# KyleVanMeter/MVOLPS

Measured on AMD Instinct MI355X. Metric: simplex_pivots_per_s, higher is better.
Workload: dtype f64

## Files before the change

mvolps_amd/csrc/engine.cpp:

```cpp
#include <hip/hip_runtime.h>

#include <cmath>
#include <cstdio>
#include <cstdlib>
#include <cstring>
#include <atomic>
#include <limits>
#include <map>
#include <mutex>
#include <tuple>
#include <unordered_map>
#include <unordered_set>
#include <vector>

#include "engine.hpp"

struct DevMatrix {
  int m0 = 0, n = 0, lda = 0;
  double *plain = nullptr, *packed = nullptr;
  int *len = nullptr;
  std::vector<const void *> rows;
  ~DevMatrix() {
    if (packed && packed != plain) (void)hipFree(packed);
    if (plain) (void)hipFree(plain);
    if (len) (void)hipFree(len);
  }
};

struct RoundModel {
  int m0 = 0, n = 0, ldm = 0, dir = 0;
  void *dev = nullptr;
  void *dev_rows = nullptr;
  int ldn = 0;
  size_t o_rlo = 0, o_rhi = 0, o_clo = 0, o_chi = 0, o_c = 0, o_flags = 0;
  std::vector<mvx::RowPtr> rows;
  std::vector<double> c, clb, cub, rlb, rub;
  std::vector<int> kind;
  ~RoundModel() {
    if (dev) (void)hipFree(dev);
    if (dev_rows) (void)hipFree(dev_rows);
  }
};

namespace mvx {

#define HIPCHECK(expr)                                                                         \
  do {                                                                                         \
    hipError_t e_ = (expr);                                                                    \
    if (e_ != hipSuccess) {                                                                    \
      std::fprintf(stderr, "mvx: HIP error %s at %s:%d (%s)\n", hipGetErrorString(e_), __FILE__, __LINE__, #expr); \
      std::abort();                                                                            \
    }                                                                                          \
  } while (0)

void set_tuning(int tr, int hot, int nt);
int fused_npb(int n);
int fused_nrb_max(int m);
int chain_ncb(int n);
int chain_nrb(int m);
void launch_pboot(const ChainArgs &, hipStream_t);
void launch_pstep(const ChainArgs &, int g, hipStream_t);
void launch_pc(const ChainArgs &, int g, hipStream_t);
void launch_fbc3(const ChainArgs &, int steps, hipStream_t);
void launch_fpatch(const ChainArgs &, int steps, hipStream_t);
int launch_chain(const ChainArgs &, hipStream_t);
int chain_cluster_nw(int m, int n);
int chain_cluster_kmax(int m, int n);
void launch_dboot(Ctl *, int n, hipStream_t);
void launch_da(Ctl *, int n, hipStream_t);
void launch_db(Ctl *, int m, int n, hipStream_t);
void launch_select(Ctl *, hipStream_t, int slots = 1);
int launch_dsel(Ctl *, int m, int n, hipStream_t, int slots = 1);
void launch_select_queue(Ctl *, const BatchQueue &q, hipStream_t, int slots);
void launch_update(Ctl *, int m, int n, hipStream_t, int slots = 1, int chained = 0, int busy_slots = 0);
void launch_p1_head(Ctl *, hipStream_t);
void launch_p1_select(Ctl *, hipStream_t);
void launch_p1_fix(Ctl *, int n, hipStream_t);
void launch_scatter_ctl(Ctl *dst, const Ctl *src, const int *idx, int count, hipStream_t);
void launch_copy_many(const CopyBatch &b, hipStream_t);
void launch_gmi(const GmiArgs &a, hipStream_t);
void launch_classify(const ClsArgs &a, hipStream_t);
void launch_penalty(const PenArgs &a, hipStream_t);
void launch_round(const RndArgs &a, hipStream_t);
void launch_rcfix(const RcArgs &a, hipStream_t);
void launch_tighten(const TightHandle *hs, const TightEntry *es, int count, hipStream_t);
void launch_prop(const PropArgs &a, hipStream_t);
void launch_setbnds(const SetbHandle *hs, const SetbEntry *es, const SetbShift *ss, int handles, hipStream_t);
void launch_refresh_select(Ctl *, const int *tflag, int var, hipStream_t);
size_t persist_lds_bytes(int m, int cpw);
int persist_max_cpw();
int persist_slot_words(int m_cap);
int launch_persist(Ctl *, unsigned long long *head, unsigned long long *slot, int *abort_flag, unsigned long long *dbg, int m, int cpw, int nw,
                   int slot_stride, int max_steps, int head_stride, hipStream_t);
void launch_rowcomb(Ctl *, int m, int n, int respect_done, hipStream_t);
void launch_shift_nonbasic(double *T, int ld, int m, int jj, double delta, hipStream_t);
void launch_set_basic_bounds(double *blb, double *bub, int i, double lb, double ub, hipStream_t);
void launch_set_nonbasic(double *nlb, double *nub, int *nflag, int j, double lb, double ub, int flag, hipStream_t);
void launch_add_rows(double *T, int ld, int n, int *bvar, double *blb, double *bub, int *nvar, int first, int nrs, int m_new,
                     hipStream_t);
void launch_export(Ctl *, unsigned char *stage, int m, int n, int force, hipStream_t, int slots = 1, size_t slot_stride = 0);

static inline size_t align_up(size_t x, size_t a) { return (x + a - 1) / a * a; }

struct Carver {
  size_t off = 0;
  size_t operator()(size_t bytes) {
    size_t o = off;
    off = align_up(off + bytes, 256);
    return o;
  }
};

constexpr size_t XG_BYTES = 4 * 8 * 64 * 16;
struct SolveCtx {
  hipStream_t stream = nullptr;
  Ctl *d_ctl = nullptr;
  Ctl *h_ctl = nullptr;
  int sc_m_cap = 0, sc_ld = 0;
  void *scratch = nullptr;
  double *d_colq = nullptr, *d_srow = nullptr, *d_cost1 = nullptr, *d_wts = nullptr, *d_part = nullptr, *d_rcbase = nullptr;
  int *d_gflag = nullptr;
  double *d_colqx[2] = {nullptr, nullptr}, *d_betac[2] = {nullptr, nullptr};
  double *d_dw = nullptr, *d_dw2 = nullptr;
  int *d_p1list = nullptr;
  int *d_tflag = nullptr;
  double *d_pw[2] = {nullptr, nullptr};
  double *d_srowk[KCH] = {}, *d_colqk[KCH] = {};
  double *d_drowk[2] = {}, *d_pwk[2] = {}, *d_nlbk[2] = {}, *d_nubk[2] = {}, *d_betak[2] = {}, *d_blbk[2] = {}, *d_bubk[2] = {};
  int *d_nflagk[2] = {};
  double *d_betab = nullptr, *d_ppart = nullptr, *d_rpart = nullptr;
  double *d_zeros = nullptr;
  unsigned char *rc_ring = nullptr;
  size_t rc_slot_bytes = 0;
  int rc_next = 0, rc_m_cap = 0, rc_ld = 0;
  unsigned *d_xg = nullptr;
  int *d_xabort = nullptr;
  unsigned xtag = 0;
  size_t pp_stride = 0, rp_stride = 0;
  size_t sk_stride = 0, ck_stride = 0;
  Cand *d_rpc = nullptr;
  double *d_olb = nullptr, *d_oub = nullptr;
  Cand *d_pp[2] = {nullptr, nullptr}, *d_rp = nullptr;
  unsigned char *d_stage = nullptr, *h_stage = nullptr;
  bool stage_zc = false;
  size_t stage_bytes = 0;
  hipEvent_t ev_a = nullptr, ev_b = nullptr;
  unsigned long long *d_pcand = nullptr, *d_pmsg = nullptr;
// ... 892 lines not shown
  if (J.parm.it_lim > 8 && J.try_fused) J.batch = std::min(J.parm.it_lim, 256);
}

static void job_enqueue(Context &c, SolveJob &J) {
  mvx_prob *P = J.P;
  SolveCtx &sc = *J.sc;
  const int m = P->m, n = P->n;
  J.ev_used = 0;
  if (J.mode == SolveJob::FINAL) {
    launch_export(sc.d_ctl, sc.d_stage, m, n, 1, sc.stream);
    stage_copy_async(sc, P);
    return;
  }
  if (J.mode == SolveJob::PHASE1) {
    for (int k = 0; k < J.pb; k++) {
      launch_p1_head(sc.d_ctl, sc.stream);
      launch_p1_fix(sc.d_ctl, n, sc.stream);
      launch_p1_select(sc.d_ctl, sc.stream);
      launch_update(sc.d_ctl, m + 1, n, sc.stream);
    }
    launch_export(sc.d_ctl, sc.d_stage, m, n, 0, sc.stream);
    stage_copy_async(sc, P);
    return;
  }
  const int batch = J.batch;
  if (J.profiled && c.ev_pool.size() < (size_t)2 * batch + 4) {
    size_t old = c.ev_pool.size();
    c.ev_pool.resize((size_t)2 * batch + 4);
    for (size_t k = old; k < c.ev_pool.size(); k++) HIPCHECK(hipEventCreate(&c.ev_pool[k]));
  }
  const int remaining = (J.parm.it_lim >= 0) ? std::max(0, J.parm.it_lim - J.seen_pivots) : (1 << 30);
  auto ev = [&]() {
    if (J.profiled) HIPCHECK(hipEventRecord(c.ev_pool[J.ev_used++], sc.stream));
  };
  int depth;
  if (J.try_fused) depth = std::max(0, std::min(batch, remaining));
  else depth = std::max(1, std::min(batch, remaining));
  auto body = [&](int m_grid) {
    if (J.try_fused) {
      PersistPlan pl;
      if (depth > 0 && !J.profiled && J.resident && !(J.cluster && !g_cluster_broken.load()) && persist_plan(c, P, &pl) && ensure_persist(c, sc, P, pl)) {
        launch_select(sc.d_ctl, sc.stream);
        launch_update(sc.d_ctl, m_grid, n, sc.stream, 1, 1);
        HIPCHECK(hipMemcpyAsync(sc.p_backup, P->slab, P->slab_bytes, hipMemcpyDeviceToDevice, sc.stream));
        HIPCHECK(hipMemcpyAsync(sc.d_pctl, sc.d_ctl, sizeof(Ctl), hipMemcpyDeviceToDevice, sc.stream));
        HIPCHECK(hipMemcpyAsync(sc.d_ppw, sc.d_pw[0], (size_t)P->ld * 8, hipMemcpyDeviceToDevice, sc.stream));
        HIPCHECK(hipMemcpyAsync(sc.d_ppw + P->ld, sc.d_pw[1], (size_t)P->ld * 8, hipMemcpyDeviceToDevice, sc.stream));
        const int head_stride = 4;
        HIPCHECK(hipMemsetAsync(sc.d_pcand, 0, (size_t)2 * pl.nw * head_stride * 8, sc.stream));
        const int steps = 1 << 24;
        if (launch_persist(sc.d_ctl, sc.d_pcand, sc.d_pmsg, sc.d_pabort, (unsigned long long *)(sc.d_pabort + 16), P->m, pl.cpw, pl.nw, sc.p_msg_words, steps, head_stride, sc.stream) == 0) {
          J.persist_queued = true;
          g_persist_launches++;
          launch_select(sc.d_ctl, sc.stream);
          launch_update(sc.d_ctl, m_grid, n, sc.stream, 1, 1);
        } else {
          g_persist_broken = true;
        }
      } else {
        const size_t e_generic = J.ev_used;
        if (J.profiled) J.ev_used += 2;
        if (depth > 0) {
          const bool cl = J.cluster && !g_cluster_broken.load();
          if (!cl) launch_pboot(J.cargs, sc.stream);
          bool first = true;
          const int kc = cl ? std::max(1, std::min(J.chain0, chain_cluster_kmax(m, n))) : std::max(1, J.chain);
          auto chain_launch = [&](int steps) {
            J.cargs.kmax = steps;
            J.cargs.boot = first ? 1 : 0;
            first = false;
            J.cargs.tagbase = sc.xtag;
            sc.xtag += 128;
            if (launch_chain(J.cargs, sc.stream) != 0) g_cluster_broken.store(true);
            g_cluster_launches++;
          };
          for (int left = depth; left > 0;) {
            const int steps = std::min(kc, left);
            if (cl) chain_launch(steps);
            else
              for (int t = 0; t < steps; t++) launch_pstep(J.cargs, t, sc.stream);
            ev();
            launch_fbc3(J.cargs, steps, sc.stream);
            ev();
            launch_fpatch(J.cargs, steps, sc.stream);
            left -= steps;
          }
          if (J.parm.it_lim >= 0 && depth >= remaining && !cl) launch_pc(J.cargs, 0, sc.stream);
        }
        launch_select(sc.d_ctl, sc.stream);
        if (J.profiled) HIPCHECK(hipEventRecord(c.ev_pool[e_generic], sc.stream));
        launch_update(sc.d_ctl, m_grid, n, sc.stream, 1, 1);
        if (J.profiled) HIPCHECK(hipEventRecord(c.ev_pool[e_generic + 1], sc.stream));
      }
    } else if (J.try_dfused) {
      launch_select(sc.d_ctl, sc.stream);
      launch_update(sc.d_ctl, m_grid, n, sc.stream, 1, 1);
      if (depth > 1) {
        launch_dboot(sc.d_ctl, n, sc.stream);
        launch_db(sc.d_ctl, m_grid, n, sc.stream);
        for (int k = 0; k < depth - 1; k++) {
          launch_da(sc.d_ctl, n, sc.stream);
          launch_db(sc.d_ctl, m_grid, n, sc.stream);
        }
      }
    } else {
      for (int k = 0; k < depth; k++) {
        launch_dsel(sc.d_ctl, m, n, sc.stream);
        launch_select(sc.d_ctl, sc.stream);
        ev();
        launch_update(sc.d_ctl, m_grid, n, sc.stream, 1, 1);
        ev();
      }
    }
    launch_export(sc.d_ctl, sc.d_stage, m_grid, n, 0, sc.stream);
    stage_copy_async(sc, P);
  };
  body(m);
}

static bool job_finalize(SolveJob &J) {
  mvx_prob *P = J.P;
  SolveCtx &sc = *J.sc;
  const Ctl &snap = J.snap;
  const unsigned char *s = sc.h_stage;
  const double *beta = (const double *)(s + sizeof(Ctl));
  const double *dj = beta + (P->m_cap + 1);
  const int *bv = (const int *)(dj + P->ld);
  const int *nv = bv + (P->m_cap + 1);
  const int *nf = nv + P->ld;
  P->beta.assign(beta, beta + P->m + 1);
  P->dj.assign(dj, dj + P->n + 1);
  P->bvar.assign(bv, bv + P->m + 1);
  P->nvar.assign(nv, nv + P->n + 1);
  P->nflag.assign(nf, nf + P->n + 1);
  rebuild_pos(P);
  P->sol_fresh = true;
  P->fresh_rows = -1;
  float ms = 0.f;
  HIPCHECK(hipEventElapsedTime(&ms, sc.ev_a, sc.ev_b));
  P->last_ms = ms;
  P->it_cnt += snap.it_cnt;
  P->bland_cnt += snap.n_bland;
  P->pert_cnt += snap.n_pert;
  P->hint_dual = false;
  switch (J.done) {
    case D_OPT: P->status = MVX_OPT; J.rc = 0; break;
    case D_UNBND: P->status = MVX_UNBND; J.rc = 0; break;
    case D_NOFEAS: P->status = MVX_NOFEAS; J.rc = 0; break;
    case D_ITLIM:
      P->status = (snap.phase == PH_PRIMAL2) ? MVX_FEAS : MVX_INFEAS;
      J.rc = MVX_EITLIM;
      break;
    default: P->status = MVX_UNDEF; J.rc = MVX_EFAIL; break;
  }
  return true;
}

static bool job_collect(Context &c, SolveJob &J) {
  SolveCtx &sc = *J.sc;
  Ctl &snap = J.snap;
  if (J.persist_queued) {
    J.persist_queued = false;
    if (sc.h_pabort[0]) {
      mvx_prob *P = J.P;
      g_persist_broken = true;
      g_persist_aborts++;
      std::fprintf(stderr, "mvx: resident-tableau launch aborted (workgroups not co-resident in time); using the two-kernel path from now on\n");
// ... 1662 lines not shown
```

mvolps_amd/csrc/kernels.hip:

```cpp
#include <hip/hip_runtime.h>

#include <cmath>
#include <cstdlib>

#include "mvx_internal.hpp"

namespace mvx {

#define TIDX ((int)threadIdx.x)

__device__ __forceinline__ double xdiv(double a, double b) {
  const double q = a / b;
  const double aq = fabs(q);
  if (!(aq > 1e-290 && aq < 1e290)) return q;
  const double r = fma(-q, b, a);
  if (r == 0.0) return q;
  const bool up = (r > 0.0) == (b > 0.0);
  long long bits = __double_as_longlong(q);
  bits += ((q > 0.0) == up) ? 1 : -1;
  const double q1 = __longlong_as_double(bits);
  const double r1 = fma(-q1, b, a);
  return (fabs(r1) < fabs(r)) ? q1 : q;
}

// ... 2628 lines not shown
      A.drowk[xf][0] = z;
      A.pwk[xf][0] = 1.0;
    }
  }
  if (lead) {
    c->pc_n = g;
    if (g > 0) {
      c->phase = PH_PRIMAL2;
      c->pc_itlim = end_itlim ? 1 : 0;
    }
  }
}

__device__ void chain_commit(const ChainArgs &A, Ctl *c, int nch) {
  __shared__ int s_cp[KCH], s_cq[KCH], s_ck[KCH], s_rf[KCH], s_cf[KCH], s_R[KCH], s_C[KCH];
  const int t = TIDX;
  const bool on = (t < nch);
  int kind = 0, p = 0, q = 0;
  if (on) {
    kind = c->ch_kind[t];
    p = c->ch_p[t];
    q = c->ch_q[t];
    s_ck[t] = kind;
    s_cp[t] = p;
    s_cq[t] = q;
    s_R[t] = (kind == ST_PIVOT) ? c->bvar[p] : 0;
    s_C[t] = (kind == ST_PIVOT) ? c->nvar[q] : 0;
  }
  __syncthreads();
  bool lastrow = true, lastcol = true, lastflag = true;
  if (on) {
    int rf = t, cf = t;
    for (int u = t - 1; u >= 0; u--) {
      if (s_ck[u] != ST_PIVOT) continue;
      if (s_cp[u] == p) rf = u;
      if (s_cq[u] == q) cf = u;
    }
    s_rf[t] = rf;
    s_cf[t] = cf;
    for (int u = t + 1; u < nch; u++) {
      if (s_cq[u] == q) lastflag = false;
      if (s_ck[u] != ST_PIVOT) continue;
      if (s_cp[u] == p) lastrow = false;
      if (s_cq[u] == q) lastcol = false;
    }
  }
  __syncthreads();
  if (t == 0) {
    for (int u = 0; u < nch; u++) {
      if (s_ck[u] != ST_PIVOT) continue;
      const int a = s_rf[u], b = s_cf[u];
      const int kv = s_R[a];
      s_R[a] = s_C[b];
      s_C[b] = kv;
    }
  }
  __syncthreads();
  if (on) {
    if (kind == ST_PIVOT) {
      if (lastrow) {
        c->bvar[p] = s_R[s_rf[t]];
        A.blb[p] = c->ch_elb[t];
        A.bub[p] = c->ch_eub[t];
      }
      if (lastcol) {
        c->nvar[q] = s_C[s_cf[t]];
        A.nlb[q] = c->ch_llb[t];
        A.nub[q] = c->ch_lub[t];
      }
    }
    if (lastflag) A.nflag[q] = c->ch_lf[t];
  }
  if (t == 0) {
    const int piv_n = c->ch_cnt[nch - 1];
    c->it_cnt += piv_n;
    c->n_flips += nch - piv_n;
    c->n_bulk++;
    if (c->budget > 0) c->budget -= piv_n;
    c->stall = c->ch_stall[nch - 1];
    c->pc_epoch++;
  }
}

typedef const double __attribute__((address_space(4))) *kconst_f64;
template <int TR, int NT>
__global__ __launch_bounds__(256) void k_fbc3(const ChainArgs A) {
  __shared__ double s_cq[KCH][TR];
  Ctl *const c = A.c;
  if (c->done != D_RUN || c->fstate != F_RUN) return;
  const int nch = c->pc_n;
  if (nch == 0) return;
  const int n = A.n;
  const size_t ld = (size_t)A.ld;
  const int j0 = 2 * ((int)blockIdx.x * 256 + TIDX);
  const int i0 = 1 + (int)blockIdx.y * TR;
  const int xf = nch & 1;
  const bool act = (j0 <= n);
  const int jc = act ? j0 : 0;
  double *base = A.T + (size_t)i0 * ld + jc;
  double2 v[TR];
#pragma unroll
  for (int r = 0; r < TR; r++) v[r] = ld2<NT>(reinterpret_cast<const double2 *>(base + (size_t)r * ld));
  unsigned flips = 0;
  for (int l = 0; l < nch; l++) flips |= (c->ch_kind[l] == ST_FLIP) ? (1u << l) : 0u;
  for (int e = TIDX; e < nch * TR; e += 256) {
    const int l = e / TR, r = e % TR;
    s_cq[l][r] = ((flips >> l) & 1u) ? 0.0 : A.colq0[(size_t)l * A.cstride + i0 + r];
  }
  __syncthreads();
  const double *sp = A.srow0 + jc;
  const double *zp = A.zeros + jc;
  for (int l0 = 0; l0 < nch; l0 += 4) {
    double2 s4[4];
#pragma unroll
    for (int k = 0; k < 4; k++) {
      const int lk = (l0 + k < nch) ? l0 + k : nch - 1;
      s4[k] = *reinterpret_cast<const double2 *>(((flips >> lk) & 1u) ? zp : sp + (size_t)lk * A.sstride);
    }
#pragma unroll
    for (int k = 0; k < 4; k++) {
      if (l0 + k < nch) {
#pragma unroll
        for (int r = 0; r < TR; r++) {
          const double ci = s_cq[l0 + k][r];
          asm("v_fma_f64 %0, -%1, %2, %0" : "+v"(v[r].x) : "v"(ci), "v"(s4[k].x));
          asm("v_fma_f64 %0, -%1, %2, %0" : "+v"(v[r].y) : "v"(ci), "v"(s4[k].y));
        }
      }
    }
  }
  if (act) {
    if (j0 == 0) {
#pragma unroll
      for (int r = 0; r < TR; r++) base[(size_t)r * ld + 1] = v[r].y;
    } else {
#pragma unroll
      for (int r = 0; r < TR; r++) st2<NT>(reinterpret_cast<double2 *>(base + (size_t)r * ld), v[r]);
    }
    if (blockIdx.y == 0) {
      *reinterpret_cast<double2 *>(A.T + j0) = *reinterpret_cast<const double2 *>(A.drowk[xf] + j0);
      const double2 w = *reinterpret_cast<const double2 *>(A.pwk[xf] + j0);
      *reinterpret_cast<double2 *>(A.pw[0] + j0) = w;
      *reinterpret_cast<double2 *>(A.pw[1] + j0) = w;
    }
  }
  if (blockIdx.x == 0 && blockIdx.y == 0) chain_commit(A, c, nch);
}

__global__ __launch_bounds__(256) void k_fpatch(const ChainArgs A, int kmax) {
  __shared__ int s_kind[KCH], s_p[KCH], s_q[KCH];
  __shared__ double s_piv[KCH], s_ip[KCH], s_xq[KCH], s_delta[KCH], s_u[KCH];
  Ctl *const c = A.c;
  if (c->done != D_RUN || c->fstate != F_RUN) return;
  const int nch = c->pc_n;
  if (nch == 0) return;
  const int m = A.m, n = A.n;
  const size_t ld = (size_t)A.ld;
  const int job = (int)blockIdx.y, x = (int)blockIdx.x * 256 + TIDX;
  const int jk = (job < kmax) ? 0 : (job < 2 * kmax) ? 1 : 2;
  const int l = (jk == 0) ? job : (jk == 1) ? job - kmax : -1;
  bool live = (jk == 2) || (l < nch && c->ch_kind[l < nch ? l : 0] == ST_PIVOT);
  const int span = (jk == 0) ? n : (jk == 1) ? m : A.mcap1 - 1;
  if ((int)blockIdx.x * 256 > span) live = false;
  if (live) {
    const int lp = (l >= 0) ? c->ch_p[l] : 0, lq = (l >= 0) ? c->ch_q[l] : 0;
    if (TIDX < KCH) {
      const int t = (TIDX < nch) ? TIDX : nch - 1;
      const int kind = c->ch_kind[t];
      const double piv = c->ch_piv[t];
      s_kind[TIDX] = kind;
      s_p[TIDX] = c->ch_p[t];
      s_q[TIDX] = c->ch_q[t];
      s_piv[TIDX] = piv;
      s_ip[TIDX] = (kind == ST_PIVOT) ? xdiv(1.0, piv) : 0.0;
      s_xq[TIDX] = c->ch_xq[t];
      s_delta[TIDX] = c->ch_delta[t];
      s_u[TIDX] = (jk == 0) ? A.colq0[(size_t)t * A.cstride + lp] : A.srow0[(size_t)t * A.sstride + (jk == 1 ? lq : 0)];
    }
    const int xc = (x >= 1 && x <= span) ? x : 1;
    double op[KCH];
#pragma unroll
    for (int t = 0; t < KCH; t++) {
      const int tc = (t < nch) ? t : nch - 1;
      op[t] = (jk == 0) ? A.srow0[(size_t)tc * A.sstride + xc] : A.colq0[(size_t)tc * A.cstride + xc];
    }
    double *dst = (jk == 0) ? A.T + (size_t)lp * ld + xc : A.T + (size_t)xc * ld + (jk == 1 ? lq : 0);
    double val = (jk == 2) ? *dst : 0.0;
    __syncthreads();
    const int i = (jk == 0) ? lp : xc, j = (jk == 0) ? xc : (jk == 1) ? lq : 0;
    const int l0 = (jk == 2) ? 0 : l;
#pragma unroll
    for (int t = 0; t < KCH; t++) {
      if (t >= l0 && t < nch) {
        const double ci = (jk == 0) ? s_u[t] : op[t], sj = (jk == 0) ? op[t] : s_u[t];
        if (s_kind[t] == ST_FLIP) {
          if (j == 0) val = fma(ci, s_delta[t], val);
        } else if (i == s_p[t]) {
          val = (j == s_q[t]) ? s_ip[t] : (j == 0) ? s_xq[t] - sj : -sj;
        } else if (j == s_q[t]) {
          val = xdiv(ci, s_piv[t]);
        } else {
          val = fma(-ci, sj, val);
        }
      }
    }
    if (x >= 1 && x <= span) {
      if (jk != 2 || x <= m) *dst = val;
      if (jk == 2) A.betab[x] = val;
    }
  }
}

__device__ __forceinline__ bool row_violation(double beta, double lb, double ub, double tol, double &viol, int &up) {
  viol = 0.0;
  up = 0;
  if (lb > -INFINITY && beta < lb - tol * (1.0 + fabs(lb))) viol = lb - beta;
  if (ub < INFINITY && beta > ub + tol * (1.0 + fabs(ub))) {
    viol = beta - ub;
    up = 1;
  }
  return viol > 0.0;
}

__device__ __forceinline__ bool dual_ratio_col(double a, double d, int f, int to_upper, double tp, int j, Cand &x) {
  if (f == MVX_NS) return false;
  const double aa = to_upper ? -a : a;
  double r;
  if (aa > tp && (f == MVX_NL || f == MVX_NF)) r = (f == MVX_NF) ? fabs(d) : (d < 0.0 ? -d : 0.0);
  else if (aa < -tp && (f == MVX_NU || f == MVX_NF)) r = (f == MVX_NF) ? fabs(d) : (d > 0.0 ? d : 0.0);
  else return false;
  const double mag = fabs(a);
  x = Cand{xdiv(r, mag), mag, j, 0};
  return true;
}

__global__ __launch_bounds__(DA_THREADS) void k_dboot(Ctl *c) {
  __shared__ Cand lds[17];
  const bool lead = (blockIdx.x == 0 && TIDX == 0);
  if (c->done != D_RUN || c->phase != PH_DUAL || c->stall >= c->stall_limit || c->perturbed) {
    if (lead) c->fstate = F_OFF;
    return;
  }
  const int a = c->curA & 1, m = c->m, n = c->n;
  const size_t ld = (size_t)c->ld;
  const double *T = c->T, *w = c->dwx[a];
  const double tol = c->tol_bnd;
  Cand rb{0.0, 0.0, 0, 0};
  for (int i = 1 + TIDX; i <= m; i += DA_THREADS) {
    double viol;
    int up;
    if (row_violation(T[(size_t)i * ld], c->blb[i], c->bub[i], tol, viol, up)) {
      Cand x{xdiv(viol * viol, w[i]), 0.0, i, up};
      if (cand_better<0>(x, rb)) rb = x;
    }
  }
  rb = block_best<0>(rb, lds);
  const int p2 = rb.idx, p2_up = rb.aux;
  const int j = (int)blockIdx.x * DA_THREADS + TIDX;
  Cand best{0.0, 0.0, 0, 0};
  if (p2 && j >= 1 && j <= n) {
    Cand x{0.0, 0.0, 0, 0};
    if (dual_ratio_col(T[(size_t)p2 * ld + j], c->sgn * T[j], c->nflag[j], p2_up, c->tol_piv, j, x)) best = x;
  }
  __syncthreads();
  best = block_best<1>(best, lds);
  if (TIDX == 0) c->pp[a][blockIdx.x] = best;
  if (lead) {
    c->p_nextx[a] = p2;
    c->p_up_nextx[a] = p2_up;
    c->fstate = F_RUN_DUAL;
    c->step = ST_NONE;
    c->curB = a ^ 1;
    c->npbd = (int)gridDim.x;
  }
}

__global__ __launch_bounds__(DA_THREADS) void k_da(Ctl *c) {
  __shared__ Cand lds[17];
  const int done = c->done, fstate = c->fstate, cur = c->curA, budget = c->budget;
  const int stall = c->stall, stall_limit = c->stall_limit;
  const int npb = c->npbd, m = c->m, n = c->n;
  const size_t ld = (size_t)c->ld;
  double *const T = c->T;
  double *const srow = c->srow;
  const int *const nflag = c->nflag;
  const double *const colq = c->colqx[cur];
  const double *const betac = c->betac[cur];
  const Cand *const pp = c->pp[cur];
  Cand *const ppn = c->pp[cur ^ 1];
  const double *const dwc = c->dwx[cur & 1];
  double *const dwn = c->dwx[(cur & 1) ^ 1];
  const double sgn = c->sgn, tol_bnd = c->tol_bnd, tol_piv = c->tol_piv;
  const int p = c->p_nextx[cur & 1], p_up = c->p_up_nextx[cur & 1];
// ... 1150 lines not shown
      h.nlb[e.idx] = e.lb;
      h.nub[e.idx] = e.ub;
      h.nflag[e.idx] = e.flag;
    }
  }
  if (h.s1 <= h.s0) return;
  for (int i = TIDX; i <= h.m; i += 256) {
    double *row = h.T + (size_t)i * (size_t)h.ld;
    double acc = row[0];
    for (int k = h.s0; k < h.s1; k++) acc = fma(row[ss[k].jj], ss[k].delta, acc);
    row[0] = acc;
  }
}

void launch_setbnds(const SetbHandle *hs, const SetbEntry *es, const SetbShift *ss, int handles, hipStream_t s) {
  hipLaunchKernelGGL(k_setbnds, dim3((unsigned)handles), dim3(256), 0, s, hs, es, ss);
}


static int g_tr = 0, g_hot = 1, g_nt = -1;
void set_tuning(int tr, int hot, int nt) {
  g_tr = (tr == 4 || tr == 8 || tr == 16 || tr == 32) ? tr : 0;
  g_hot = hot ? 1 : 0;
  g_nt = (nt >= 0 && nt <= 2) ? nt : -1;
}
static int pick_nt(int m, int n) {
  if (g_nt >= 0) return g_nt;
  const size_t bytes = (size_t)(m + 1) * (size_t)((n + 1 + LD_ALIGN - 1) / LD_ALIGN * LD_ALIGN) * 8;
  if (bytes > NT_THRESHOLD_BYTES) return 1;
  return (bytes >= WT_MIN_BYTES && bytes <= WT_MAX_BYTES) ? 2 : 0;
}
static int pick_tr(int m, int n) {
  if (g_tr) return g_tr;
  const long tiles = ((n + 2) / 2 + 255) / 256;
  if ((long)((m + 15) / 16) * tiles >= 2048) return 16;
  if ((long)((m + 7) / 8) * tiles >= 2048) return 8;
  return 4;
}
int fused_npb(int n) { return (n + 1 + 255) / 256; }
int fused_nrb_max(int m) { return (m + 3) / 4; }
int chain_ncb(int n) { return fused_npb(n); }
int chain_nrb(int m) { return (m + 255) / 256; }
void launch_pboot(const ChainArgs &a, hipStream_t s) {
  hipLaunchKernelGGL(k_pboot, dim3(a.ncb > a.nrb ? a.ncb : a.nrb), dim3(256), 0, s, a);
}
void launch_pstep(const ChainArgs &a, int g, hipStream_t s) {
  hipLaunchKernelGGL(k_pc, dim3(a.nrb), dim3(256), 0, s, a, g);
  hipLaunchKernelGGL(k_pr, dim3(a.ncb), dim3(256), 0, s, a, g);
}
void launch_pc(const ChainArgs &a, int g, hipStream_t s) { hipLaunchKernelGGL(k_pc, dim3(a.nrb), dim3(256), 0, s, a, g); }
int chain_cluster_nw(int m, int n) {
  const int span = m > n ? m : n;
  int nw = (span + 255) / 256;
  if (nw > 32) nw = 32;
  return nw < 1 ? 1 : nw;
}
int chain_cluster_kmax(int m, int n) {
  const int nw = chain_cluster_nw(m, n), tt = nw * 256;
  const int cpt = (n + tt - 1) / tt, rpt = (m + tt - 1) / tt;
  if (cpt > 2 || rpt > 2) return 0;
  const int per_step = (cpt > 1 || rpt > 1 ? 4 : 2) * 256 * 8;
  const int k = (140 * 1024) / per_step;
  return k > KCH ? KCH : k;
}
int launch_chain(const ChainArgs &a, hipStream_t s) {
  const int tt = a.nw * 256;
  const int cpt = (a.n + tt - 1) / tt, rpt = (a.m + tt - 1) / tt;
  const bool wide = (cpt > 1 || rpt > 1);
  const size_t lds = (size_t)(a.kmax > 0 ? a.kmax : 1) * (wide ? 4 : 2) * 256 * 8;
  static size_t attr1 = 0, attr2 = 0;
  size_t &attr = wide ? attr2 : attr1;
  const void *fn = wide ? reinterpret_cast<const void *>(k_chain<2, 2>) : reinterpret_cast<const void *>(k_chain<1, 1>);
  if (lds > attr) {
    if (hipFuncSetAttribute(fn, hipFuncAttributeMaxDynamicSharedMemorySize, (int)lds) != hipSuccess) {
      (void)hipGetLastError();
      return -1;
    }
    attr = lds;
  }
  if (wide) hipLaunchKernelGGL((k_chain<2, 2>), dim3(8 * a.nw), dim3(256), lds, s, a);
  else hipLaunchKernelGGL((k_chain<1, 1>), dim3(8 * a.nw), dim3(256), lds, s, a);
  return 0;
}
void launch_fpatch(const ChainArgs &a, int steps, hipStream_t s) {
  const int span = a.mcap1 > a.n + 1 ? a.mcap1 : a.n + 1;
  hipLaunchKernelGGL(k_fpatch, dim3((span + 255) / 256, 2 * steps + 1), dim3(256), 0, s, a, steps);
}
void launch_fbc3(const ChainArgs &a, int steps, hipStream_t s) {
  const int m = a.m, n = a.n;
  const int pairs = (n + 2) / 2;
  int tr = pick_tr(m, n);
  if (tr > 16) tr = 16;
  if (!g_tr && tr == 16 && steps >= 12) tr = 8;
  const int nt = pick_nt(m, n);
  dim3 grid((pairs + 255) / 256, (m + tr - 1) / tr);
#define FBC2_CASE(TR_, NT_) \
  if (tr == TR_ && nt == NT_) { hipLaunchKernelGGL((k_fbc3<TR_, NT_>), grid, dim3(256), 0, s, a); return; }
  FBC2_CASE(16, 0) FBC2_CASE(16, 1) FBC2_CASE(16, 2) FBC2_CASE(8, 0) FBC2_CASE(8, 1) FBC2_CASE(8, 2) FBC2_CASE(4, 0) FBC2_CASE(4, 1) FBC2_CASE(4, 2)
#undef FBC2_CASE
  std::abort();
}
void launch_dboot(Ctl *d_ctl, int n, hipStream_t s) { hipLaunchKernelGGL(k_dboot, dim3((n + DA_THREADS) / DA_THREADS), dim3(DA_THREADS), 0, s, d_ctl); }
void launch_da(Ctl *d_ctl, int n, hipStream_t s) { hipLaunchKernelGGL(k_da, dim3((n + DA_THREADS) / DA_THREADS), dim3(DA_THREADS), 0, s, d_ctl); }
void launch_db(Ctl *d_ctl, int m, int n, hipStream_t s) {
  const int pairs = (n + 2) / 2;
  const int tr = pick_tr(m, n);
  const int nt = pick_nt(m, n);
  dim3 grid((pairs + 255) / 256, (m + tr - 1) / tr);
#define DB_CASE(TR_, NT_) \
  if (tr == TR_ && nt == NT_) { hipLaunchKernelGGL((k_fb<TR_, 1, NT_, 1>), grid, dim3(256), 0, s, d_ctl); return; }
  DB_CASE(16, 0) DB_CASE(16, 1) DB_CASE(8, 0) DB_CASE(8, 1) DB_CASE(4, 0) DB_CASE(4, 1) DB_CASE(32, 0) DB_CASE(32, 1)
  DB_CASE(16, 2) DB_CASE(8, 2) DB_CASE(4, 2) DB_CASE(32, 2)
#undef DB_CASE
  std::abort();
}
int launch_dsel(Ctl *d_ctl, int m, int n, hipStream_t s, int slots) {
  static int state = -1;
  if (state < 0) {
    const char *e = std::getenv("MVX_DSEL");
    if (e && e[0] == '0') state = 0;
    else if (hipFuncSetAttribute(reinterpret_cast<const void *>(k_dsel), hipFuncAttributeMaxDynamicSharedMemorySize, (int)DSEL_LDS) == hipSuccess) state = 1;
    else {
      (void)hipGetLastError();
      state = 0;
    }
  }
  if (state != 1 || m > 1024 || n > 1024) return 0;
  hipLaunchKernelGGL(k_dsel, dim3(1, 1, slots), dim3(1024), DSEL_LDS, s, d_ctl);
  return 1;
}
void launch_select(Ctl *d_ctl, hipStream_t s, int slots) {
  BatchQueue q{};
  hipLaunchKernelGGL(k_select, dim3(1, 1, slots), dim3(1024), 0, s, d_ctl, q);
}
void launch_select_queue(Ctl *d_ctl, const BatchQueue &q, hipStream_t s, int slots) {
  hipLaunchKernelGGL(k_select, dim3(1, 1, slots), dim3(1024), 0, s, d_ctl, q);
}
void launch_update(Ctl *d_ctl, int m, int n, hipStream_t s, int slots, int chained, int busy_slots) {
  const int pairs = (n + 2) / 2;
  const long tiles = (pairs + 255) / 256;
  const long work = busy_slots > 0 ? std::min(busy_slots, slots) : slots;
  int tr = ((long)((m + 16) / 16) * tiles * work >= 2048) ? 16 : ((long)((m + 8) / 8) * tiles * work >= 2048) ? 8 : 4;
  static const int tr_cap = std::getenv("MVX_UPD_TR") ? std::atoi(std::getenv("MVX_UPD_TR")) : 4;
  if (slots > 1 && chained && tr > tr_cap) tr = tr_cap >= 16 ? 16 : tr_cap >= 8 ? 8 : 4;
  dim3 grid((unsigned)tiles, (m + tr) / tr, slots);
  const int nt = (tr == 16) ? pick_nt(m, n) : 0;
  if (nt == 1) hipLaunchKernelGGL((k_update<16, 1>), grid, dim3(256), 0, s, d_ctl, chained);
  else if (nt == 2) hipLaunchKernelGGL((k_update<16, 2>), grid, dim3(256), 0, s, d_ctl, chained);
  else if (tr == 16) hipLaunchKernelGGL((k_update<16, 0>), grid, dim3(256), 0, s, d_ctl, chained);
  else if (tr == 8) hipLaunchKernelGGL((k_update<8, 0>), grid, dim3(256), 0, s, d_ctl, chained);
  else hipLaunchKernelGGL((k_update<4, 0>), grid, dim3(256), 0, s, d_ctl, chained);
}
void launch_p1_head(Ctl *d_ctl, hipStream_t s) { hipLaunchKernelGGL(k_p1_head, dim3(1), dim3(1024), 0, s, d_ctl); }
void launch_p1_select(Ctl *d_ctl, hipStream_t s) { hipLaunchKernelGGL(k_p1_select, dim3(1), dim3(1024), 0, s, d_ctl); }
__global__ __launch_bounds__(64) void k_scatter_ctl(Ctl *dst, const Ctl *src, const int *idx, int count) {
  const int t = (int)blockIdx.x;
  if (t >= count) return;
  const unsigned *s = reinterpret_cast<const unsigned *>(&src[t]);
  unsigned *d = reinterpret_cast<unsigned *>(&dst[idx[t]]);
  for (int w = TIDX; w < (int)(sizeof(Ctl) / 4); w += 64) d[w] = s[w];
}
void launch_scatter_ctl(Ctl *dst, const Ctl *src, const int *idx, int count, hipStream_t s) {
  hipLaunchKernelGGL(k_scatter_ctl, dim3(count), dim3(64), 0, s, dst, src, idx, count);
}
__global__ __launch_bounds__(256) void k_copy_many(CopyBatch b) {
  const CopyJob j = b.jobs[blockIdx.y];
  const uint4 *__restrict__ src = reinterpret_cast<const uint4 *>(j.src);
  uint4 *__restrict__ dst = reinterpret_cast<uint4 *>(j.dst);
  const size_t n = j.bytes >> 4;
  constexpr int U = 8;
  for (size_t base = (size_t)blockIdx.x * (256 * U); base < n; base += (size_t)gridDim.x * (256 * U)) {
    uint4 v[U];
#pragma unroll
    for (int u = 0; u < U; u++) {
      const size_t i = base + (size_t)u * 256 + TIDX;
      if (i < n) v[u] = src[i];
    }
#pragma unroll
    for (int u = 0; u < U; u++) {
      const size_t i = base + (size_t)u * 256 + TIDX;
// ... 41 lines not shown
```

Before: 58570.

## Fuse fpatch into fbc3 launch and stage chain operands in LDS

Drops the separate patch kernel and folds its jobs into the leading blocks of a single 1-D grid for the bulk chained update, saving one launch per chain segment. The bulk blocks now cover 64 column pairs by four waves of rows and stage the pivot-row and pivot-column operands into dynamic shared memory, so the data is reused across waves instead of each thread re-reading it from global memory. Rows and columns that the patch jobs rewrite are masked out with wave ballots, which avoids write races between the two job types in the same launch. The patch jobs also skip loading operand groups below their starting step. The cost is more complex indexing and a dependence on the patch blocks and bulk blocks touching disjoint elements within one launch.

```diff
diff --git a/mvolps_amd/csrc/engine.cpp b/mvolps_amd/csrc/engine.cpp
--- a/mvolps_amd/csrc/engine.cpp
+++ b/mvolps_amd/csrc/engine.cpp
@@ -62,7 +62,6 @@
 void launch_pstep(const ChainArgs &, int g, hipStream_t);
 void launch_pc(const ChainArgs &, int g, hipStream_t);
 void launch_fbc3(const ChainArgs &, int steps, hipStream_t);
-void launch_fpatch(const ChainArgs &, int steps, hipStream_t);
 int launch_chain(const ChainArgs &, hipStream_t);
 int chain_cluster_nw(int m, int n);
 int chain_cluster_kmax(int m, int n);
@@ -1121,7 +1120,6 @@
             ev();
             launch_fbc3(J.cargs, steps, sc.stream);
             ev();
-            launch_fpatch(J.cargs, steps, sc.stream);
             left -= steps;
           }
           if (J.parm.it_lim >= 0 && depth >= remaining && !cl) launch_pc(J.cargs, 0, sc.stream);
diff --git a/mvolps_amd/csrc/kernels.hip b/mvolps_amd/csrc/kernels.hip
--- a/mvolps_amd/csrc/kernels.hip
+++ b/mvolps_amd/csrc/kernels.hip
@@ -2734,133 +2734,197 @@
   }
 }
 
-typedef const double __attribute__((address_space(4))) *kconst_f64;
+__device__ void fpatch_job(const ChainArgs &A, Ctl *c, int nch, int kmax, int job, int bx) {
+  __shared__ int s_kind[KCH], s_p[KCH], s_q[KCH];
+  __shared__ double s_piv[KCH], s_ip[KCH], s_xq[KCH], s_delta[KCH], s_u[KCH];
+  const int m = A.m, n = A.n;
+  const size_t ld = (size_t)A.ld;
+  const int x = bx * 256 + TIDX;
+  const int jk = (job < kmax) ? 0 : (job < 2 * kmax) ? 1 : 2;
+  const int l = (jk == 0) ? job : (jk == 1) ? job - kmax : -1;
+  bool live = (jk == 2) || (l < nch && c->ch_kind[l < nch ? l : 0] == ST_PIVOT);
+  const int span = (jk == 0) ? n : (jk == 1) ? m : A.mcap1 - 1;
+  if (bx * 256 > span) live = false;
+  if (!live) return;
+  const int lp = (l >= 0) ? c->ch_p[l] : 0, lq = (l >= 0) ? c->ch_q[l] : 0;
+  if (TIDX < KCH) {
+    const int t = (TIDX < nch) ? TIDX : nch - 1;
+    const int kind = c->ch_kind[t];
+    const double piv = c->ch_piv[t];
+    s_kind[TIDX] = kind;
+    s_p[TIDX] = c->ch_p[t];
+    s_q[TIDX] = c->ch_q[t];
+    s_piv[TIDX] = piv;
+    s_ip[TIDX] = (kind == ST_PIVOT) ? xdiv(1.0, piv) : 0.0;
+    s_xq[TIDX] = c->ch_xq[t];
+    s_delta[TIDX] = c->ch_delta[t];
+    s_u[TIDX] = (jk == 0) ? A.colq0[(size_t)t * A.cstride + lp] : A.srow0[(size_t)t * A.sstride + (jk == 1 ? lq : 0)];
+  }
+  const int xc = (x >= 1 && x <= span) ? x : 1;
+  const int l0 = (jk == 2) ? 0 : l;
+  double op[KCH];
+#pragma unroll
+  for (int t = 0; t < KCH; t++) op[t] = 0.0;
+#pragma unroll
+  for (int g = 0; g < KCH / 8; g++) {
+    if (g >= l0 / 8 && g * 8 < nch) {
+#pragma unroll
+      for (int u = 0; u < 8; u++) {
+        const int t = g * 8 + u, tc = (t < nch) ? t : nch - 1;
+        op[t] = (jk == 0) ? A.srow0[(size_t)tc * A.sstride + xc] : A.colq0[(size_t)tc * A.cstride + xc];
+      }
+    }
+  }
+  double *dst = (jk == 0) ? A.T + (size_t)lp * ld + xc : A.T + (size_t)xc * ld + (jk == 1 ? lq : 0);
+  double val = (jk == 2) ? *dst : 0.0;
+  __syncthreads();
+  const int i = (jk == 0) ? lp : xc, j = (jk == 0) ? xc : (jk == 1) ? lq : 0;
+#pragma unroll
+  for (int t = 0; t < KCH; t++) {
+    if (t >= l0 && t < nch) {
+      const double ci = (jk == 0) ? s_u[t] : op[t], sj = (jk == 0) ? op[t] : s_u[t];
+      if (s_kind[t] == ST_FLIP) {
+        if (j == 0) val = fma(ci, s_delta[t], val);
+      } else if (i == s_p[t]) {
+        val = (j == s_q[t]) ? s_ip[t] : (j == 0) ? s_xq[t] - sj : -sj;
+      } else if (j == s_q[t]) {
+        val = xdiv(ci, s_piv[t]);
+      } else {
+        val = fma(-ci, sj, val);
+      }
+    }
+  }
+  if (x >= 1 && x <= span) {
+    if (jk != 2 || x <= m) *dst = val;
+    if (jk == 2) A.betab[x] = val;
+  }
+}
+
+constexpr int FBC_LANES = 64;
+constexpr int fbc3_ng(int steps) { return steps <= 4 ? 1 : steps <= 8 ? 2 : steps <= 16 ? 4 : KCH / 4; }
+constexpr int fbc3_nc(int tr, int ng) { return (ng * tr + 15) / 16; }
+constexpr int fbc3_lds_bytes(int tr, int steps) { return 4 * fbc3_ng(steps) * FBC_LANES * 16 + fbc3_nc(tr, fbc3_ng(steps)) * 256 * 8; }
+template <int TR, int NG>
+__device__ __forceinline__ void fbc3_stage(const ChainArgs &A, double2 *sr, int nch, unsigned flips, int jb, int ib) {
+  constexpr int WR = 4 * TR, NC = fbc3_nc(TR, NG);
+  double *const cq = reinterpret_cast<double *>(sr + 4 * NG * FBC_LANES);
+  double2 ts[NG];
+  double tc[NC];
+#pragma unroll
+  for (int k = 0; k < NG; k++) {
+    const int e = k * 256 + TIDX, l = e / FBC_LANES;
+    const int lc = (l < nch) ? l : nch - 1;
+    const int j = jb + 2 * (e % FBC_LANES);
+    const int jc = (j <= A.n) ? j : 0;
+    ts[k] = *reinterpret_cast<const double2 *>((((flips >> lc) & 1u) ? A.zeros : A.srow0 + (size_t)lc * A.sstride) + jc);
+  }
+#pragma unroll
+  for (int k = 0; k < NC; k++) {
+    const int e = k * 256 + TIDX, l = e / WR;
+    const int lc = (l < nch) ? l : nch - 1;
+    const int i = ib + e % WR;
+    const int ic = (i < A.mcap1) ? i : A.mcap1 - 1;
+    tc[k] = (((flips >> lc) & 1u) ? A.zeros : A.colq0 + (size_t)lc * A.cstride)[ic];
+  }
+#pragma unroll
+  for (int k = 0; k < NG; k++) sr[k * 256 + TIDX] = ts[k];
+#pragma unroll
+  for (int k = 0; k < NC; k++) cq[k * 256 + TIDX] = tc[k];
+}
 template <int TR, int NT>
-__global__ __launch_bounds__(256) void k_fbc3(const ChainArgs A) {
-  __shared__ double s_cq[KCH][TR];
+__global__ __launch_bounds__(256) void k_fbc3(const ChainArgs A, int kmax, int npx, int nx) {
+  extern __shared__ double2 s_ops[];
   Ctl *const c = A.c;
   if (c->done != D_RUN || c->fstate != F_RUN) return;
   const int nch = c->pc_n;
   if (nch == 0) return;
+  const int npatch = npx * (2 * kmax + 1);
+  if ((int)blockIdx.x < npatch) {
+    fpatch_job(A, c, nch, kmax, (int)blockIdx.x / npx, (int)blockIdx.x % npx);
+    return;
+  }
+  const int bx = ((int)blockIdx.x - npatch) % nx, by = ((int)blockIdx.x - npatch) / nx;
   const int n = A.n;
   const size_t ld = (size_t)A.ld;
-  const int j0 = 2 * ((int)blockIdx.x * 256 + TIDX);
-  const int i0 = 1 + (int)blockIdx.y * TR;
+  const int lane = TIDX & 63, w = TIDX >> 6;
+  const int jb = 2 * bx * FBC_LANES, j0 = jb + 2 * lane;
+  const int ib = 1 + by * 4 * TR, i0 = ib + w * TR;
   const int xf = nch & 1;
   const bool act = (j0 <= n);
+  const bool rows = (i0 <= A.m);
   const int jc = act ? j0 : 0;
-  double *base = A.T + (size_t)i0 * ld + jc;
+  double *base = A.T + (size_t)(rows ? i0 : 1) * ld + jc;
+  const int lt = lane < nch ? lane : nch - 1;
+  const int kind = c->ch_kind[lt], pl = c->ch_p[lt], ql = c->ch_q[lt];
   double2 v[TR];
 #pragma unroll
   for (int r = 0; r < TR; r++) v[r] = ld2<NT>(reinterpret_cast<const double2 *>(base + (size_t)r * ld));
-  unsigned flips = 0;
-  for (int l = 0; l < nch; l++) flips |= (c->ch_kind[l] == ST_FLIP) ? (1u << l) : 0u;
-  for (int e = TIDX; e < nch * TR; e += 256) {
-    const int l = e / TR, r = e % TR;
-    s_cq[l][r] = ((flips >> l) & 1u) ? 0.0 : A.colq0[(size_t)l * A.cstride + i0 + r];
-  }
+  const unsigned flips = (unsigned)__ballot(lane < nch && kind == ST_FLIP);
+  const bool piv = (lane < nch) && kind == ST_PIVOT;
+  unsigned rowmask = 0;
+#pragma unroll
+  for (int r = 0; r < TR; r++) rowmask |= (__ballot(piv && pl == i0 + r) != 0ull) ? (1u << r) : 0u;
+  unsigned long long cm = __ballot(piv && ql >= jb && ql < jb + 2 * FBC_LANES);
+  const bool part = (cm != 0ull) || (bx == 0);
+  bool skx = (j0 == 0), sky = false;
+  while (cm != 0ull) {
+    const int q = __builtin_amdgcn_readlane(ql, (int)__builtin_ctzll(cm));
+    cm &= cm - 1;
+    skx = skx || (q == j0);
+    sky = sky || (q == j0 + 1);
+  }
+  double2 *const s_sr = s_ops;
+  const double *s_cq;
+  if (nch <= 4) fbc3_stage<TR, 1>(A, s_sr, nch, flips, jb, ib), s_cq = reinterpret_cast<const double *>(s_sr + 4 * FBC_LANES);
+  else if (nch <= 8) fbc3_stage<TR, 2>(A, s_sr, nch, flips, jb, ib), s_cq = reinterpret_cast<const double *>(s_sr + 8 * FBC_LANES);
+  else if (nch <= 16) fbc3_stage<TR, 4>(A, s_sr, nch, flips, jb, ib), s_cq = reinterpret_cast<const double *>(s_sr + 16 * FBC_LANES);
+  else fbc3_stage<TR, KCH / 4>(A, s_sr, nch, flips, jb, ib), s_cq = reinterpret_cast<const double *>(s_sr + KCH * FBC_LANES);
   __syncthreads();
-  const double *sp = A.srow0 + jc;
-  const double *zp = A.zeros + jc;
+  const double2 *sp = s_sr + lane;
+  const double *cp = s_cq + w * TR;
   for (int l0 = 0; l0 < nch; l0 += 4) {
     double2 s4[4];
 #pragma unroll
     for (int k = 0; k < 4; k++) {
       const int lk = (l0 + k < nch) ? l0 + k : nch - 1;
-      s4[k] = *reinterpret_cast<const double2 *>(((flips >> lk) & 1u) ? zp : sp + (size_t)lk * A.sstride);
+      s4[k] = sp[lk * FBC_LANES];
     }
 #pragma unroll
     for (int k = 0; k < 4; k++) {
       if (l0 + k < nch) {
 #pragma unroll
         for (int r = 0; r < TR; r++) {
-          const double ci = s_cq[l0 + k][r];
+          const double ci = cp[(l0 + k) * 4 * TR + r];
           asm("v_fma_f64 %0, -%1, %2, %0" : "+v"(v[r].x) : "v"(ci), "v"(s4[k].x));
           asm("v_fma_f64 %0, -%1, %2, %0" : "+v"(v[r].y) : "v"(ci), "v"(s4[k].y));
         }
       }
     }
   }
-  if (act) {
-    if (j0 == 0) {
-#pragma unroll
-      for (int r = 0; r < TR; r++) base[(size_t)r * ld + 1] = v[r].y;
+  if (act && rows) {
+    if (!part) {
+#pragma unroll
+      for (int r = 0; r < TR; r++)
+        if (!((rowmask >> r) & 1u)) st2<NT>(reinterpret_cast<double2 *>(base + (size_t)r * ld), v[r]);
     } else {
 #pragma unroll
-      for (int r = 0; r < TR; r++) st2<NT>(reinterpret_cast<double2 *>(base + (size_t)r * ld), v[r]);
-    }
-    if (blockIdx.y == 0) {
-      *reinterpret_cast<double2 *>(A.T + j0) = *reinterpret_cast<const double2 *>(A.drowk[xf] + j0);
-      const double2 w = *reinterpret_cast<const double2 *>(A.pwk[xf] + j0);
-      *reinterpret_cast<double2 *>(A.pw[0] + j0) = w;
-      *reinterpret_cast<double2 *>(A.pw[1] + j0) = w;
-    }
-  }
-  if (blockIdx.x == 0 && blockIdx.y == 0) chain_commit(A, c, nch);
-}
-
-__global__ __launch_bounds__(256) void k_fpatch(const ChainArgs A, int kmax) {
-  __shared__ int s_kind[KCH], s_p[KCH], s_q[KCH];
-  __shared__ double s_piv[KCH], s_ip[KCH], s_xq[KCH], s_delta[KCH], s_u[KCH];
-  Ctl *const c = A.c;
-  if (c->done != D_RUN || c->fstate != F_RUN) return;
-  const int nch = c->pc_n;
-  if (nch == 0) return;
-  const int m = A.m, n = A.n;
-  const size_t ld = (size_t)A.ld;
-  const int job = (int)blockIdx.y, x = (int)blockIdx.x * 256 + TIDX;
-  const int jk = (job < kmax) ? 0 : (job < 2 * kmax) ? 1 : 2;
-  const int l = (jk == 0) ? job : (jk == 1) ? job - kmax : -1;
-  bool live = (jk == 2) || (l < nch && c->ch_kind[l < nch ? l : 0] == ST_PIVOT);
-  const int span = (jk == 0) ? n : (jk == 1) ? m : A.mcap1 - 1;
-  if ((int)blockIdx.x * 256 > span) live = false;
-  if (live) {
-    const int lp = (l >= 0) ? c->ch_p[l] : 0, lq = (l >= 0) ? c->ch_q[l] : 0;
-    if (TIDX < KCH) {
-      const int t = (TIDX < nch) ? TIDX : nch - 1;
-      const int kind = c->ch_kind[t];
-      const double piv = c->ch_piv[t];
-      s_kind[TIDX] = kind;
-      s_p[TIDX] = c->ch_p[t];
-      s_q[TIDX] = c->ch_q[t];
-      s_piv[TIDX] = piv;
-      s_ip[TIDX] = (kind == ST_PIVOT) ? xdiv(1.0, piv) : 0.0;
-      s_xq[TIDX] = c->ch_xq[t];
-      s_delta[TIDX] = c->ch_delta[t];
-      s_u[TIDX] = (jk == 0) ? A.colq0[(size_t)t * A.cstride + lp] : A.srow0[(size_t)t * A.sstride + (jk == 1 ? lq : 0)];
-    }
-    const int xc = (x >= 1 && x <= span) ? x : 1;
-    double op[KCH];
-#pragma unroll
-    for (int t = 0; t < KCH; t++) {
-      const int tc = (t < nch) ? t : nch - 1;
-      op[t] = (jk == 0) ? A.srow0[(size_t)tc * A.sstride + xc] : A.colq0[(size_t)tc * A.cstride + xc];
-    }
-    double *dst = (jk == 0) ? A.T + (size_t)lp * ld + xc : A.T + (size_t)xc * ld + (jk == 1 ? lq : 0);
-    double val = (jk == 2) ? *dst : 0.0;
-    __syncthreads();
-    const int i = (jk == 0) ? lp : xc, j = (jk == 0) ? xc : (jk == 1) ? lq : 0;
-    const int l0 = (jk == 2) ? 0 : l;
-#pragma unroll
-    for (int t = 0; t < KCH; t++) {
-      if (t >= l0 && t < nch) {
-        const double ci = (jk == 0) ? s_u[t] : op[t], sj = (jk == 0) ? op[t] : s_u[t];
-        if (s_kind[t] == ST_FLIP) {
-          if (j == 0) val = fma(ci, s_delta[t], val);
-        } else if (i == s_p[t]) {
-          val = (j == s_q[t]) ? s_ip[t] : (j == 0) ? s_xq[t] - sj : -sj;
-        } else if (j == s_q[t]) {
-          val = xdiv(ci, s_piv[t]);
-        } else {
-          val = fma(-ci, sj, val);
+      for (int r = 0; r < TR; r++) {
+        if ((rowmask >> r) & 1u) continue;
+        if (!skx && !sky) st2<NT>(reinterpret_cast<double2 *>(base + (size_t)r * ld), v[r]);
+        else {
+          if (!skx) base[(size_t)r * ld] = v[r].x;
+          if (!sky) base[(size_t)r * ld + 1] = v[r].y;
         }
       }
     }
-    if (x >= 1 && x <= span) {
-      if (jk != 2 || x <= m) *dst = val;
-      if (jk == 2) A.betab[x] = val;
-    }
-  }
+  }
+  if (act && by == 0 && w == 0) {
+    *reinterpret_cast<double2 *>(A.T + j0) = *reinterpret_cast<const double2 *>(A.drowk[xf] + j0);
+    const double2 w2 = *reinterpret_cast<const double2 *>(A.pwk[xf] + j0);
+    *reinterpret_cast<double2 *>(A.pw[0] + j0) = w2;
+    *reinterpret_cast<double2 *>(A.pw[1] + j0) = w2;
+  }
+  if (bx == 0 && by == 0) chain_commit(A, c, nch);
 }
 
 __device__ __forceinline__ bool row_violation(double beta, double lb, double ub, double tol, double &viol, int &up) {
@@ -4177,10 +4241,6 @@
   else hipLaunchKernelGGL((k_chain<1, 1>), dim3(8 * a.nw), dim3(256), lds, s, a);
   return 0;
 }
-void launch_fpatch(const ChainArgs &a, int steps, hipStream_t s) {
-  const int span = a.mcap1 > a.n + 1 ? a.mcap1 : a.n + 1;
-  hipLaunchKernelGGL(k_fpatch, dim3((span + 255) / 256, 2 * steps + 1), dim3(256), 0, s, a, steps);
-}
 void launch_fbc3(const ChainArgs &a, int steps, hipStream_t s) {
   const int m = a.m, n = a.n;
   const int pairs = (n + 2) / 2;
@@ -4188,9 +4248,12 @@
   if (tr > 16) tr = 16;
   if (!g_tr && tr == 16 && steps >= 12) tr = 8;
   const int nt = pick_nt(m, n);
-  dim3 grid((pairs + 255) / 256, (m + tr - 1) / tr);
+  const int span = a.mcap1 > n + 1 ? a.mcap1 : n + 1;
+  const int npx = (span + 255) / 256, nx = (pairs + FBC_LANES - 1) / FBC_LANES, ny = (m + 4 * tr - 1) / (4 * tr);
+  dim3 grid((unsigned)(npx * (2 * steps + 1) + nx * ny));
+  const int lds = fbc3_lds_bytes(tr, steps < 1 ? 1 : steps);
 #define FBC2_CASE(TR_, NT_) \
-  if (tr == TR_ && nt == NT_) { hipLaunchKernelGGL((k_fbc3<TR_, NT_>), grid, dim3(256), 0, s, a); return; }
+  if (tr == TR_ && nt == NT_) { hipLaunchKernelGGL((k_fbc3<TR_, NT_>), grid, dim3(256), lds, s, a, steps, npx, nx); return; }
   FBC2_CASE(16, 0) FBC2_CASE(16, 1) FBC2_CASE(16, 2) FBC2_CASE(8, 0) FBC2_CASE(8, 1) FBC2_CASE(8, 2) FBC2_CASE(4, 0) FBC2_CASE(4, 1) FBC2_CASE(4, 2)
 #undef FBC2_CASE
   std::abort();
```

After: 57540. -1.8%, worse.
